# MaxInGaussian/SCFGP

Measured on AMD Instinct MI355X. Metric: NLML+grad evals/sec, higher is better.
Workload: dtype f32

## Files before the change

scfgp_amd/csrc/apply_epilogue.h:

```cpp
#pragma once
#include "kernels.h"
#include "tile_cfgs.h"

template <int CTRL> __device__ __forceinline__ double dpp_mov_f64(double x) {
    int lo = __double2loint(x), hi = __double2hiint(x);
    lo = __builtin_amdgcn_update_dpp(0, lo, CTRL, 0xF, 0xF, true);
    hi = __builtin_amdgcn_update_dpp(0, hi, CTRL, 0xF, 0xF, true);
    return __hiloint2double(hi, lo);
}
__device__ __forceinline__ double row16_sum(double x) {
    x += dpp_mov_f64<0xB1>(x);
    x += dpp_mov_f64<0x4E>(x);
    x += dpp_mov_f64<0x141>(x);
    x += dpp_mov_f64<0x140>(x);
    return x;
}
template <class Cfg, int EPI, bool MU>
__device__ __forceinline__ void apply_epilogue_vec2(
    const typename Cfg::MTr::acc_t (&acc)[Cfg::TM][Cfg::TN], const double* __restrict__ Phi, double* V,
    double* __restrict__ vpart, const double* __restrict__ p, const double* __restrict__ q, const double* __restrict__ y,
    const double* __restrict__ alpha, const double* __restrict__ ut, int K, int Kp, int64_t Np, int64_t rb, int cbase, int jtg,
    char* smem_raw, double* __restrict__ mupart, int tid) {
    static_assert(Cfg::TN == 2 && Cfg::MS == 16 && sizeof(typename Cfg::T) == 8 && (EPI == 0 || EPI == 1 || EPI == 3 || EPI == 4), "VEC2 layout");
    AccCoord<Cfg> co(tid);
    const int jg = cbase + co.wn0 + 2 * (co.lane & 15);
    if constexpr (EPI == 4) {
#pragma unroll
        for (int tm = 0; tm < Cfg::TM; ++tm)
#pragma unroll
            for (int r = 0; r < 4; ++r)
                *reinterpret_cast<v2d*>(V + (rb * Cfg::BM + co.row(tm, r)) * Kp + jg) = v2d{acc[tm][0][r], acc[tm][1][r]};
    } else if constexpr (EPI == 0 || EPI == 3) {
        double* red = reinterpret_cast<double*>(smem_raw);
        double* red2 = red + Cfg::WGN * Cfg::BM;
        const int wn = (tid >> 6) % Cfg::WGN;
        double al[2], live[2];
#pragma unroll
        for (int k = 0; k < 2; ++k) { live[k] = jg + k < K ? 1.0 : 0.0; al[k] = MU && jg + k < K ? alpha[jg + k] : 0.0; }
#pragma unroll
        for (int tm = 0; tm < Cfg::TM; ++tm) {
            v2d ph[4];
            int64_t off[4];
#pragma unroll
            for (int r = 0; r < 4; ++r) {
                off[r] = (rb * Cfg::BM + co.row(tm, r)) * Kp + jg;
                if (EPI == 0) ph[r] = *reinterpret_cast<const v2d*>(Phi + off[r]);
            }
#pragma unroll
            for (int r = 0; r < 4; ++r) {
                const int row = co.row(tm, r);
                const double c0 = acc[tm][0][r], c1 = acc[tm][1][r];
                *reinterpret_cast<v2d*>(V + off[r]) = v2d{c0, c1};
                double part, mup = 0;
                if (EPI == 3) part = fma(c0, c0, c1 * c1);
                else part = fma(ph[r][0] * live[0], c0, ph[r][1] * live[1] * c1);
                if (MU) mup = EPI == 3 ? fma(c0, al[0], c1 * al[1]) : fma(ph[r][0], al[0], ph[r][1] * al[1]);
                part = row16_sum(part);
                if ((co.lane & 15) == 0) red[wn * Cfg::BM + row] = part;
                if (MU) {
                    mup = row16_sum(mup);
                    if ((co.lane & 15) == 0) red2[wn * Cfg::BM + row] = mup;
                }
            }
        }
        __syncthreads();
        if (tid < Cfg::BM) {
            double s = 0, s2 = 0;
#pragma unroll
            for (int k = 0; k < Cfg::WGN; ++k) { s += red[k * Cfg::BM + tid]; if (MU) s2 += red2[k * Cfg::BM + tid]; }
            vpart[(int64_t)jtg * Np + rb * Cfg::BM + tid] = s;
            if (MU && mupart) mupart[(int64_t)jtg * Np + rb * Cfg::BM + tid] = s2;
        }
    } else {
        double al[2], u2[2];
#pragma unroll
        for (int k = 0; k < 2; ++k) { al[k] = alpha[jg + k]; u2[k] = ut[jg + k]; }
        double* rowsc = reinterpret_cast<double*>(smem_raw);
        for (int i = tid; i < Cfg::BM; i += Cfg::THREADS) {
            const int64_t n = rb * Cfg::BM + i;
            rowsc[3 * i] = 2.0 * q[n]; rowsc[3 * i + 1] = p[n]; rowsc[3 * i + 2] = y[n];
        }
        __syncthreads();
#pragma unroll
        for (int tm = 0; tm < Cfg::TM; ++tm) {
            v2d vv[4];
            int64_t off[4];
#pragma unroll
            for (int r = 0; r < 4; ++r) {
                off[r] = (rb * Cfg::BM + co.row(tm, r)) * Kp + jg;
                vv[r] = *reinterpret_cast<const v2d*>(V + off[r]);
            }
#pragma unroll
            for (int r = 0; r < 4; ++r) {
                const int row = co.row(tm, r);
                const double qn = rowsc[3 * row], pn = rowsc[3 * row + 1], yn = rowsc[3 * row + 2];
                v2d o;
#pragma unroll
                for (int k = 0; k < 2; ++k) o[k] = 2.0 * acc[tm][k][r] + qn * vv[r][k] + pn * al[k] + yn * u2[k];
                *reinterpret_cast<v2d*>(V + off[r]) = o;
            }
        }
    }
}
template <class Cfg, int EPI, bool MU = false, bool VEC4 = false>
__device__ __forceinline__ void apply_epilogue(
    const typename Cfg::MTr::acc_t (&acc)[Cfg::TM][Cfg::TN], const typename Cfg::T* __restrict__ Phi, typename Cfg::T* V,
    double* __restrict__ vpart, const double* __restrict__ p, const double* __restrict__ q, const double* __restrict__ y,
    const double* __restrict__ alpha, const double* __restrict__ ut, int K, int Kp, int64_t Np, int64_t rb, int cbase, int jtg,
    char* smem_raw, double* __restrict__ mupart = nullptr, int tid = (int)threadIdx.x) {
    typedef typename Cfg::T T;
    if constexpr (VEC4 && sizeof(T) == 8) {
        apply_epilogue_vec2<Cfg, EPI, MU>(acc, Phi, V, vpart, p, q, y, alpha, ut, K, Kp, Np, rb, cbase, jtg, smem_raw, mupart, tid);
        return;
    }
    AccCoord<Cfg> co(tid);
    if constexpr (VEC4 && sizeof(T) == 4) {
        static_assert(Cfg::TN == 4 && Cfg::MS == 16 && sizeof(T) == 4 && (EPI == 0 || EPI == 1 || EPI == 3 || EPI == 4), "VEC4 layout");
        const int c4 = co.wn0 + 4 * (co.lane & 15);
        const int jg = cbase + c4;
        if constexpr (EPI == 4) {
#pragma unroll
            for (int tm = 0; tm < Cfg::TM; ++tm)
#pragma unroll
                for (int r = 0; r < 4; ++r)
                    *reinterpret_cast<v4f*>(V + (rb * Cfg::BM + co.row(tm, r)) * Kp + jg) = v4f{acc[tm][0][r], acc[tm][1][r], acc[tm][2][r], acc[tm][3][r]};
        } else if constexpr (EPI == 0 || EPI == 3) {
            double* red = reinterpret_cast<double*>(smem_raw);
            double* red2 = red + Cfg::WGN * Cfg::BM;
            const int wn = (tid >> 6) % Cfg::WGN;
            double al[4], live[4];
#pragma unroll
            for (int k = 0; k < 4; ++k) { live[k] = jg + k < K ? 1.0 : 0.0; al[k] = MU && jg + k < K ? alpha[jg + k] : 0.0; }
#pragma unroll
            for (int tm = 0; tm < Cfg::TM; ++tm) {
                v4f ph[4];
                int64_t off[4];
#pragma unroll
                for (int r = 0; r < 4; ++r) {
                    off[r] = (rb * Cfg::BM + co.row(tm, r)) * Kp + jg;
                    if (EPI == 0) ph[r] = *reinterpret_cast<const v4f*>(Phi + off[r]);
                }
#pragma unroll
                for (int r = 0; r < 4; ++r) {
                    const int row = co.row(tm, r);
                    const v4f c = v4f{acc[tm][0][r], acc[tm][1][r], acc[tm][2][r], acc[tm][3][r]};
                    *reinterpret_cast<v4f*>(V + off[r]) = c;
                    double part = 0, mup = 0;
                    if (EPI == 3) {
                        part = (double)(c[0] * c[0]) + (double)(c[1] * c[1]) + (double)(c[2] * c[2]) + (double)(c[3] * c[3]);
                        if (MU) mup = (double)c[0] * al[0] + (double)c[1] * al[1] + (double)c[2] * al[2] + (double)c[3] * al[3];
                    } else {
#pragma unroll
                        for (int k = 0; k < 4; ++k) { part += (double)ph[r][k] * (double)c[k] * live[k]; if (MU) mup += (double)ph[r][k] * al[k]; }
                    }
                    part = row16_sum(part);
                    if ((co.lane & 15) == 0) red[wn * Cfg::BM + row] = part;
                    if (MU) {
                        mup = row16_sum(mup);
                        if ((co.lane & 15) == 0) red2[wn * Cfg::BM + row] = mup;
                    }
                }
            }
            __syncthreads();
            if (tid < Cfg::BM) {
                double s = 0, s2 = 0;
#pragma unroll
                for (int k = 0; k < Cfg::WGN; ++k) { s += red[k * Cfg::BM + tid]; if (MU) s2 += red2[k * Cfg::BM + tid]; }
                vpart[(int64_t)jtg * Np + rb * Cfg::BM + tid] = s;
                if (MU && mupart) mupart[(int64_t)jtg * Np + rb * Cfg::BM + tid] = s2;
            }
        } else {
            float alf[4], u4f[4];
#pragma unroll
            for (int k = 0; k < 4; ++k) { alf[k] = (float)alpha[jg + k]; u4f[k] = (float)ut[jg + k]; }
            float* rowsc = reinterpret_cast<float*>(smem_raw);
            for (int i = tid; i < Cfg::BM; i += Cfg::THREADS) {
                const int64_t n = rb * Cfg::BM + i;
                rowsc[3 * i] = (float)(2.0 * q[n]); rowsc[3 * i + 1] = (float)p[n]; rowsc[3 * i + 2] = (float)y[n];
            }
            __syncthreads();
#pragma unroll
            for (int tm = 0; tm < Cfg::TM; ++tm) {
                v4f vv[4];
                int64_t off[4];
#pragma unroll
                for (int r = 0; r < 4; ++r) {
                    off[r] = (rb * Cfg::BM + co.row(tm, r)) * Kp + jg;
                    vv[r] = *reinterpret_cast<const v4f*>(V + off[r]);
                }
#pragma unroll
                for (int r = 0; r < 4; ++r) {
                    const int row = co.row(tm, r);
                    const float qn = rowsc[3 * row], pn = rowsc[3 * row + 1], yn = rowsc[3 * row + 2];
                    v4f o;
#pragma unroll
                    for (int k = 0; k < 4; ++k) o[k] = fmaf(qn, vv[r][k], fmaf(pn, alf[k], fmaf(yn, u4f[k], 2.0f * acc[tm][k][r])));
                    *reinterpret_cast<v4f*>(V + off[r]) = o;
                }
            }
        }
        return;
    }
    if (EPI == 4) {
#pragma unroll
        for (int tm = 0; tm < Cfg::TM; ++tm)
#pragma unroll
            for (int r = 0; r < Cfg::MTr::NACC; ++r) {
                const int64_t off = (rb * Cfg::BM + co.row(tm, r)) * Kp + cbase;
#pragma unroll
                for (int tn = 0; tn < Cfg::TN; ++tn) V[off + co.col(tn)] = acc[tm][tn][r];
            }
    } else if (EPI == 0 || EPI == 2 || EPI == 3) {
        double* red = reinterpret_cast<double*>(smem_raw);
        double* red2 = red + Cfg::WGN * Cfg::BM;
        const int wn = (tid >> 6) % Cfg::WGN;
        double al[Cfg::TN];
        if (MU) {
#pragma unroll
            for (int tn = 0; tn < Cfg::TN; ++tn) al[tn] = cbase + co.col(tn) < K ? alpha[cbase + co.col(tn)] : 0.0;
        }
#pragma unroll
        for (int tm = 0; tm < Cfg::TM; ++tm)
#pragma unroll
            for (int r = 0; r < Cfg::MTr::NACC; ++r) {
                const int row = co.row(tm, r);
                const int64_t off = (rb * Cfg::BM + row) * Kp + cbase;
                double part = 0, mup = 0;
#pragma unroll
                for (int tn = 0; tn < Cfg::TN; ++tn) {
                    const T c = acc[tm][tn][r];
                    if (EPI != 2) V[off + co.col(tn)] = c;
                    if (EPI != 0) {
                        part += (double)c * (double)c;
                        if (MU && cbase + co.col(tn) < K) mup += (EPI == 3 ? (double)c : (double)Phi[off + co.col(tn)]) * al[tn];
                    } else if (cbase + co.col(tn) < K) {
                        const double ph = (double)Phi[off + co.col(tn)];
                        part += ph * (double)c;
                        if (MU) mup += ph * al[tn];
                    }
                }
                if constexpr (Cfg::MS == 16) part = row16_sum(part);
                else {
#pragma unroll
                    for (int m = 1; m < Cfg::MS; m <<= 1) part += __shfl_xor(part, m);
                }
                if ((co.lane % Cfg::MS) == 0) red[wn * Cfg::BM + row] = part;
                if (MU) {
                    if constexpr (Cfg::MS == 16) mup = row16_sum(mup);
                    else {
#pragma unroll
                        for (int m = 1; m < Cfg::MS; m <<= 1) mup += __shfl_xor(mup, m);
                    }
                    if ((co.lane % Cfg::MS) == 0) red2[wn * Cfg::BM + row] = mup;
                }
            }
        __syncthreads();
        if (tid < Cfg::BM) {
            double s = 0, s2 = 0;
#pragma unroll
            for (int k = 0; k < Cfg::WGN; ++k) { s += red[k * Cfg::BM + tid]; if (MU) s2 += red2[k * Cfg::BM + tid]; }
            vpart[(int64_t)jtg * Np + rb * Cfg::BM + tid] = s;
            if (MU && mupart) mupart[(int64_t)jtg * Np + rb * Cfg::BM + tid] = s2;
        }
    } else {
        [[maybe_unused]] float alf[Cfg::TN], utf[Cfg::TN];
        if constexpr (sizeof(T) == 4) {
#pragma unroll
            for (int tn = 0; tn < Cfg::TN; ++tn) { alf[tn] = (float)alpha[cbase + co.col(tn)]; utf[tn] = (float)ut[cbase + co.col(tn)]; }
        }
#pragma unroll
        for (int tm = 0; tm < Cfg::TM; ++tm)
#pragma unroll
            for (int r = 0; r < Cfg::MTr::NACC; ++r) {
                const int64_t n = rb * Cfg::BM + co.row(tm, r);
                const int64_t off = n * Kp + cbase;
                const double qn = 2.0 * q[n], pn = p[n], yn = y[n];
                if constexpr (sizeof(T) == 4) {
                    const float qf = (float)qn, pf = (float)pn, yf = (float)yn;
#pragma unroll
                    for (int tn = 0; tn < Cfg::TN; ++tn)
                        V[off + co.col(tn)] = fmaf(qf, V[off + co.col(tn)], fmaf(pf, alf[tn], fmaf(yf, utf[tn], 2.0f * acc[tm][tn][r])));
                } else {
#pragma unroll
                    for (int tn = 0; tn < Cfg::TN; ++tn) {
                        const int j = cbase + co.col(tn);
                        V[off + co.col(tn)] = (T)(2.0 * (double)acc[tm][tn][r] + qn * (double)V[off + co.col(tn)] + pn * alpha[j] + yn * ut[j]);
                    }
                }
            }
    }
}
```

Measured before the change: 4.954.

## Replace per-row DPP reductions with butterfly scatter-reduce and double-buffer V loads

The vec2/vec4 epilogue reductions used to run a full 16-lane DPP reduction for every (tm, r) row, with only lane 0 writing. They now use a transpose-style butterfly: each DPP step halves the number of live values, so all 16 lanes finish holding a distinct row's sum and each lane writes one shared-memory slot. This cuts DPP and add instruction count about 4x. The EPI 1 update path also uses 32-bit byte offsets from a block base pointer and prefetches the V tiles two tm steps ahead to overlap loads. These changes add the constraint TM==4 and raise register pressure from the double-buffered V values.

New measurement: 4.952 (median of 3 runs). About the same (-0.0%).

```diff
diff --git a/scfgp_amd/csrc/apply_epilogue.h b/scfgp_amd/csrc/apply_epilogue.h
--- a/scfgp_amd/csrc/apply_epilogue.h
+++ b/scfgp_amd/csrc/apply_epilogue.h
@@ -15,13 +15,32 @@
     x += dpp_mov_f64<0x140>(x);
     return x;
 }
+struct RowScatter {
+    bool hi[4];
+    __device__ __forceinline__ explicit RowScatter(int lane) {
+        const bool b0 = lane & 1, b1 = lane & 2, b2 = lane & 4, b3 = lane & 8;
+        hi[0] = b0 != b2; hi[1] = b1 != b2; hi[2] = b2 != b3; hi[3] = b3;
+    }
+    template <int CTRL, int N>
+    __device__ __forceinline__ static void step(double (&x)[4], bool h) {
+#pragma unroll
+        for (int i = 0; i < N / 2; ++i) {
+            const double keep = h ? x[2 * i + 1] : x[2 * i], send = h ? x[2 * i] : x[2 * i + 1];
+            x[i] = keep + dpp_mov_f64<CTRL>(send);
+        }
+    }
+    __device__ __forceinline__ double quad(double (&x)[4]) const { step<0xB1, 4>(x, hi[0]); step<0x4E, 4>(x, hi[1]); return x[0]; }
+    __device__ __forceinline__ double finish(double (&x)[4]) const { step<0x141, 4>(x, hi[2]); step<0x140, 4>(x, hi[3]); return x[0]; }
+    __device__ __forceinline__ int tm() const { return (int)hi[2] + 2 * (int)hi[3]; }
+    __device__ __forceinline__ int r() const { return (int)hi[0] + 2 * (int)hi[1]; }
+};
 template <class Cfg, int EPI, bool MU>
 __device__ __forceinline__ void apply_epilogue_vec2(
     const typename Cfg::MTr::acc_t (&acc)[Cfg::TM][Cfg::TN], const double* __restrict__ Phi, double* V,
     double* __restrict__ vpart, const double* __restrict__ p, const double* __restrict__ q, const double* __restrict__ y,
     const double* __restrict__ alpha, const double* __restrict__ ut, int K, int Kp, int64_t Np, int64_t rb, int cbase, int jtg,
     char* smem_raw, double* __restrict__ mupart, int tid) {
-    static_assert(Cfg::TN == 2 && Cfg::MS == 16 && sizeof(typename Cfg::T) == 8 && (EPI == 0 || EPI == 1 || EPI == 3 || EPI == 4), "VEC2 layout");
+    static_assert(Cfg::TM == 4 && Cfg::TN == 2 && Cfg::MS == 16 && sizeof(typename Cfg::T) == 8 && (EPI == 0 || EPI == 1 || EPI == 3 || EPI == 4), "VEC2 layout");
     AccCoord<Cfg> co(tid);
     const int jg = cbase + co.wn0 + 2 * (co.lane & 15);
     if constexpr (EPI == 4) {
@@ -37,10 +56,13 @@
         double al[2], live[2];
 #pragma unroll
         for (int k = 0; k < 2; ++k) { live[k] = jg + k < K ? 1.0 : 0.0; al[k] = MU && jg + k < K ? alpha[jg + k] : 0.0; }
+        const RowScatter rs(co.lane);
+        double partq[4], mupq[4];
 #pragma unroll
         for (int tm = 0; tm < Cfg::TM; ++tm) {
             v2d ph[4];
             int64_t off[4];
+            double part[4], mup[4];
 #pragma unroll
             for (int r = 0; r < 4; ++r) {
                 off[r] = (rb * Cfg::BM + co.row(tm, r)) * Kp + jg;
@@ -48,21 +70,18 @@
             }
 #pragma unroll
             for (int r = 0; r < 4; ++r) {
-                const int row = co.row(tm, r);
                 const double c0 = acc[tm][0][r], c1 = acc[tm][1][r];
                 *reinterpret_cast<v2d*>(V + off[r]) = v2d{c0, c1};
-                double part, mup = 0;
-                if (EPI == 3) part = fma(c0, c0, c1 * c1);
-                else part = fma(ph[r][0] * live[0], c0, ph[r][1] * live[1] * c1);
-                if (MU) mup = EPI == 3 ? fma(c0, al[0], c1 * al[1]) : fma(ph[r][0], al[0], ph[r][1] * al[1]);
-                part = row16_sum(part);
-                if ((co.lane & 15) == 0) red[wn * Cfg::BM + row] = part;
-                if (MU) {
-                    mup = row16_sum(mup);
-                    if ((co.lane & 15) == 0) red2[wn * Cfg::BM + row] = mup;
-                }
-            }
-        }
+                if (EPI == 3) part[r] = fma(c0, c0, c1 * c1);
+                else part[r] = fma(ph[r][0] * live[0], c0, ph[r][1] * live[1] * c1);
+                if (MU) mup[r] = EPI == 3 ? fma(c0, al[0], c1 * al[1]) : fma(ph[r][0], al[0], ph[r][1] * al[1]);
+            }
+            partq[tm] = rs.quad(part);
+            if (MU) mupq[tm] = rs.quad(mup);
+        }
+        const int row = co.row(rs.tm(), rs.r());
+        red[wn * Cfg::BM + row] = rs.finish(partq);
+        if (MU) red2[wn * Cfg::BM + row] = rs.finish(mupq);
         __syncthreads();
         if (tid < Cfg::BM) {
             double s = 0, s2 = 0;
@@ -81,24 +100,27 @@
             rowsc[3 * i] = 2.0 * q[n]; rowsc[3 * i + 1] = p[n]; rowsc[3 * i + 2] = y[n];
         }
         __syncthreads();
+        char* vb = reinterpret_cast<char*>(V + rb * Cfg::BM * Kp + cbase);
+        const int c2 = co.wn0 + 2 * (co.lane & 15);
+        const auto voff = [&](int tm, int r) { return (unsigned)((co.row(tm, r) * Kp + c2) * (int)sizeof(double)); };
+        v2d vv[2][4];
+        const auto vload = [&](int tm) {
+#pragma unroll
+            for (int r = 0; r < 4; ++r) vv[tm & 1][r] = *reinterpret_cast<const v2d*>(vb + voff(tm, r));
+        };
+        vload(0); vload(1);
 #pragma unroll
         for (int tm = 0; tm < Cfg::TM; ++tm) {
-            v2d vv[4];
-            int64_t off[4];
-#pragma unroll
-            for (int r = 0; r < 4; ++r) {
-                off[r] = (rb * Cfg::BM + co.row(tm, r)) * Kp + jg;
-                vv[r] = *reinterpret_cast<const v2d*>(V + off[r]);
-            }
 #pragma unroll
             for (int r = 0; r < 4; ++r) {
                 const int row = co.row(tm, r);
                 const double qn = rowsc[3 * row], pn = rowsc[3 * row + 1], yn = rowsc[3 * row + 2];
                 v2d o;
 #pragma unroll
-                for (int k = 0; k < 2; ++k) o[k] = 2.0 * acc[tm][k][r] + qn * vv[r][k] + pn * al[k] + yn * u2[k];
-                *reinterpret_cast<v2d*>(V + off[r]) = o;
-            }
+                for (int k = 0; k < 2; ++k) o[k] = 2.0 * acc[tm][k][r] + qn * vv[tm & 1][r][k] + pn * al[k] + yn * u2[k];
+                *reinterpret_cast<v2d*>(vb + voff(tm, r)) = o;
+            }
+            if (tm + 2 < Cfg::TM) vload(tm + 2);
         }
     }
 }
@@ -115,7 +137,7 @@
     }
     AccCoord<Cfg> co(tid);
     if constexpr (VEC4 && sizeof(T) == 4) {
-        static_assert(Cfg::TN == 4 && Cfg::MS == 16 && sizeof(T) == 4 && (EPI == 0 || EPI == 1 || EPI == 3 || EPI == 4), "VEC4 layout");
+        static_assert(Cfg::TM == 4 && Cfg::TN == 4 && Cfg::MS == 16 && sizeof(T) == 4 && (EPI == 0 || EPI == 1 || EPI == 3 || EPI == 4), "VEC4 layout");
         const int c4 = co.wn0 + 4 * (co.lane & 15);
         const int jg = cbase + c4;
         if constexpr (EPI == 4) {
@@ -131,10 +153,13 @@
             double al[4], live[4];
 #pragma unroll
             for (int k = 0; k < 4; ++k) { live[k] = jg + k < K ? 1.0 : 0.0; al[k] = MU && jg + k < K ? alpha[jg + k] : 0.0; }
+            const RowScatter rs(co.lane);
+            double partq[4], mupq[4];
 #pragma unroll
             for (int tm = 0; tm < Cfg::TM; ++tm) {
                 v4f ph[4];
                 int64_t off[4];
+                double part[4], mup[4];
 #pragma unroll
                 for (int r = 0; r < 4; ++r) {
                     off[r] = (rb * Cfg::BM + co.row(tm, r)) * Kp + jg;
@@ -142,25 +167,23 @@
                 }
 #pragma unroll
                 for (int r = 0; r < 4; ++r) {
-                    const int row = co.row(tm, r);
                     const v4f c = v4f{acc[tm][0][r], acc[tm][1][r], acc[tm][2][r], acc[tm][3][r]};
                     *reinterpret_cast<v4f*>(V + off[r]) = c;
-                    double part = 0, mup = 0;
+                    part[r] = 0; mup[r] = 0;
                     if (EPI == 3) {
-                        part = (double)(c[0] * c[0]) + (double)(c[1] * c[1]) + (double)(c[2] * c[2]) + (double)(c[3] * c[3]);
-                        if (MU) mup = (double)c[0] * al[0] + (double)c[1] * al[1] + (double)c[2] * al[2] + (double)c[3] * al[3];
+                        part[r] = (double)(c[0] * c[0]) + (double)(c[1] * c[1]) + (double)(c[2] * c[2]) + (double)(c[3] * c[3]);
+                        if (MU) mup[r] = (double)c[0] * al[0] + (double)c[1] * al[1] + (double)c[2] * al[2] + (double)c[3] * al[3];
                     } else {
 #pragma unroll
-                        for (int k = 0; k < 4; ++k) { part += (double)ph[r][k] * (double)c[k] * live[k]; if (MU) mup += (double)ph[r][k] * al[k]; }
+                        for (int k = 0; k < 4; ++k) { part[r] += (double)ph[r][k] * (double)c[k] * live[k]; if (MU) mup[r] += (double)ph[r][k] * al[k]; }
                     }
-                    part = row16_sum(part);
-                    if ((co.lane & 15) == 0) red[wn * Cfg::BM + row] = part;
-                    if (MU) {
-                        mup = row16_sum(mup);
-                        if ((co.lane & 15) == 0) red2[wn * Cfg::BM + row] = mup;
-                    }
-                }
-            }
+                }
+                partq[tm] = rs.quad(part);
+                if (MU) mupq[tm] = rs.quad(mup);
+            }
+            const int row = co.row(rs.tm(), rs.r());
+            red[wn * Cfg::BM + row] = rs.finish(partq);
+            if (MU) red2[wn * Cfg::BM + row] = rs.finish(mupq);
             __syncthreads();
             if (tid < Cfg::BM) {
                 double s = 0, s2 = 0;
@@ -179,24 +202,26 @@
                 rowsc[3 * i] = (float)(2.0 * q[n]); rowsc[3 * i + 1] = (float)p[n]; rowsc[3 * i + 2] = (float)y[n];
             }
             __syncthreads();
+            char* vb = reinterpret_cast<char*>(V + rb * Cfg::BM * Kp + cbase);
+            const auto voff = [&](int tm, int r) { return (unsigned)((co.row(tm, r) * Kp + c4) * (int)sizeof(float)); };
+            v4f vv[2][4];
+            const auto vload = [&](int tm) {
+#pragma unroll
+                for (int r = 0; r < 4; ++r) vv[tm & 1][r] = *reinterpret_cast<const v4f*>(vb + voff(tm, r));
+            };
+            vload(0); vload(1);
 #pragma unroll
             for (int tm = 0; tm < Cfg::TM; ++tm) {
-                v4f vv[4];
-                int64_t off[4];
-#pragma unroll
-                for (int r = 0; r < 4; ++r) {
-                    off[r] = (rb * Cfg::BM + co.row(tm, r)) * Kp + jg;
-                    vv[r] = *reinterpret_cast<const v4f*>(V + off[r]);
-                }
 #pragma unroll
                 for (int r = 0; r < 4; ++r) {
                     const int row = co.row(tm, r);
                     const float qn = rowsc[3 * row], pn = rowsc[3 * row + 1], yn = rowsc[3 * row + 2];
                     v4f o;
 #pragma unroll
-                    for (int k = 0; k < 4; ++k) o[k] = fmaf(qn, vv[r][k], fmaf(pn, alf[k], fmaf(yn, u4f[k], 2.0f * acc[tm][k][r])));
-                    *reinterpret_cast<v4f*>(V + off[r]) = o;
-                }
+                    for (int k = 0; k < 4; ++k) o[k] = fmaf(qn, vv[tm & 1][r][k], fmaf(pn, alf[k], fmaf(yn, u4f[k], 2.0f * acc[tm][k][r])));
+                    *reinterpret_cast<v4f*>(vb + voff(tm, r)) = o;
+                }
+                if (tm + 2 < Cfg::TM) vload(tm + 2);
             }
         }
         return;
```
